# brendel-group/cl-ica

Hardware: AMD Instinct MI355X
Metric: training steps/sec (B=6144, n=10 MLP) (higher is better)
Workload: dtype f32 via f16x2 split (3 fp16 MFMA products of scaled two-piece operands, fp32 accumulate)

## Files before the change

cl_ica_amd/_lib.py:

```python
from __future__ import annotations

import ctypes as C
import os
import weakref
from typing import Dict, List, Optional, Tuple

import torch

_HERE = os.path.dirname(os.path.abspath(__file__))
LIB_PATH = os.environ.get("CLICA_LIB") or os.path.join(_HERE, "lib", "libclica_hip.so")

c_f32p = C.c_void_p
c_i64 = C.c_int64
c_i32 = C.c_int32
c_size = C.c_size_t


class LpLossDesc(C.Structure):
    _fields_ = [("B", c_i64), ("B3", c_i64), ("n", c_i32), ("p", C.c_float), ("tau", C.c_float),
                ("alpha", C.c_float), ("compat", c_i32), ("pow", c_i32), ("no_eps", c_i32)]


class AdamDesc(C.Structure):
    _fields_ = [("param", C.c_void_p), ("grad", C.c_void_p), ("exp_avg", C.c_void_p), ("exp_avg_sq", C.c_void_p), ("count", c_i64),
# ... 62 lines not shown
                                 c_f32p, c_i64, c_f32p, c_i64, C.c_void_p, c_size, C.c_void_p],
    "clica_dot_loss_bwd_sym_train": [C.POINTER(DotLossDesc), c_f32p, c_i64, c_f32p, c_i64, c_f32p, c_f32p, c_f32p, c_i64, c_f32p, C.c_void_p,
                                     C.c_void_p, c_size, C.c_void_p],
    "clica_linear_fwd": [c_f32p, c_i64, c_f32p, c_i64, c_f32p, c_f32p, c_i64, c_i64, c_i64, c_i64, c_i32, C.c_float, C.c_void_p],
    "clica_linear_dgrad": [c_f32p, c_i64, c_f32p, c_i64, c_f32p, c_i64, C.c_float, c_f32p, c_i64, c_i64, c_i64, c_i64, C.c_void_p],
    "clica_linear_wgrad_workspace_bytes": [c_i64, c_i64, c_i64, C.POINTER(c_size)],
    "clica_linear_plan": [c_i32, c_i64, c_i64, c_i64, C.POINTER(c_i32), C.POINTER(c_i32), C.POINTER(c_i32), C.POINTER(c_i32)],
    "clica_linear_wgrad": [c_f32p, c_i64, c_f32p, c_i64, c_f32p, c_i64, c_f32p, c_i64, c_i64, c_i64, c_i32, C.c_void_p, c_size, C.c_void_p],
    "clica_mlp_fwd": [c_f32p, c_i64, c_i64, c_i32, C.POINTER(C.c_void_p), C.POINTER(c_i64), C.POINTER(C.c_void_p),
                      C.POINTER(C.c_void_p), C.POINTER(c_i64), C.POINTER(c_i32), C.POINTER(c_i32), c_f32p, C.POINTER(C.c_void_p), C.c_float, C.c_void_p],
    "clica_mlp_fwd_mixed": [c_f32p, c_i64, c_i64, c_f32p, c_i32, C.c_float, c_f32p, c_i64, c_i32,
                            C.POINTER(C.c_void_p), C.POINTER(c_i64), C.POINTER(C.c_void_p),
                            C.POINTER(C.c_void_p), C.POINTER(c_i64), C.POINTER(c_i32), C.POINTER(c_i32), c_f32p, C.POINTER(C.c_void_p),
                            C.c_float, C.c_void_p],
    "clica_mlp_signmask_bytes": [c_i64, C.POINTER(c_size)],
    "clica_mlp_pack_split_bytes": [c_i32, C.POINTER(c_i32), C.POINTER(c_i32), c_i32, C.POINTER(c_size)],
    "clica_mlp_pack_split": [c_i32, C.POINTER(C.c_void_p), C.POINTER(c_i64), C.POINTER(c_i32), C.POINTER(c_i32), c_i32, C.c_void_p, C.c_void_p],
    "clica_mlp_pack_split_both": [c_i32, C.POINTER(C.c_void_p), C.POINTER(c_i64), C.POINTER(c_i32), C.POINTER(c_i32), C.c_void_p, C.c_void_p,
                                  C.c_void_p],
    "clica_mlp_planes_bytes": [c_i64, c_i32, c_i32, C.POINTER(c_size)],
    "clica_mlp_fwd_split": [c_f32p, c_i64, c_i64, c_f32p, c_i32, C.c_float, c_f32p, c_i64, c_i32, C.POINTER(C.c_void_p),
                            C.POINTER(C.c_void_p), C.POINTER(c_i64), C.POINTER(c_i32), C.POINTER(c_i32), C.c_void_p, C.POINTER(C.c_void_p),
                            C.POINTER(C.c_void_p), C.c_float, C.c_void_p],
    "clica_mlp_dgrad_split": [c_f32p, c_i64, c_i64, c_i32, C.POINTER(c_i32), C.POINTER(c_i32), C.c_void_p, C.POINTER(C.c_void_p),
                              C.POINTER(C.c_void_p), C.POINTER(c_i64), C.POINTER(C.c_void_p), C.c_float, C.c_void_p],
    "clica_mlp_wgrad_split_kind": [c_i32, c_i32, C.POINTER(c_i32)],
    "clica_mlp_planes_from_f32": [c_f32p, c_i64, c_i64, c_i32, c_i32, C.c_void_p, C.c_void_p],
    "clica_mlp_planes_from_f32_t": [c_f32p, c_i64, c_i64, c_i32, C.c_void_p, C.c_void_p],
    "clica_linear_split_fwd": [C.c_void_p, C.c_void_p, c_f32p, c_i64, c_i32, c_i32, c_i32, C.c_float, C.c_void_p, C.c_void_p, c_i32,
                               c_f32p, c_i64, C.c_void_p],
    "clica_linear_split_dgrad": [C.c_void_p, C.c_void_p, C.c_void_p, C.c_float, c_i64, c_i32, c_i32, C.c_void_p, C.c_void_p,
                                 c_f32p, c_i64, C.c_void_p],
    "clica_mlp_wgrad_split_workspace_bytes": [c_i64, c_i32, C.POINTER(c_i32), C.POINTER(c_i32), C.POINTER(c_size)],
    "clica_mlp_wgrad_split": [c_i64, c_i32, C.POINTER(C.c_void_p), C.POINTER(C.c_void_p), C.POINTER(C.c_void_p), C.POINTER(c_i64),
                              C.POINTER(C.c_void_p), C.POINTER(c_i64), C.POINTER(C.c_void_p), C.POINTER(c_i64), C.POINTER(C.c_void_p),
                              C.POINTER(c_i32), C.POINTER(c_i32), c_i32, C.c_void_p, c_size, C.c_void_p],
    "clica_split16_state_bytes": [C.POINTER(c_size)],
    "clica_split16_state_init": [C.c_void_p, C.c_void_p],
    "clica_split16_update": [C.c_void_p, c_i32, C.c_void_p],
    "clica_split16_read": [C.c_void_p, C.POINTER(c_i32), C.POINTER(c_i32), c_f32p, c_f32p, c_f32p, c_f32p, c_f32p, C.c_void_p],
    "clica_split16_clear_flags": [C.c_void_p, C.c_void_p],
    "clica_split16_guard": [C.c_void_p, C.POINTER(c_i32), C.POINTER(c_i32), C.POINTER(c_i32), C.POINTER(c_i32), C.c_void_p],
    "clica_split16_set_dp_poison": [C.c_void_p, C.c_void_p, C.c_void_p],
    "clica_split16_poison_export": [C.c_void_p, C.c_void_p, C.c_void_p],
    "clica_mlp_planes16_bytes": [c_i64, c_i32, c_i32, C.POINTER(c_size)],
    "clica_mlp_pack_split16_bytes": [c_i32, C.POINTER(c_i32), C.POINTER(c_i32), c_i32, C.POINTER(c_size)],
    "clica_mlp_pack_split16_both": [c_i32, C.POINTER(C.c_void_p), C.POINTER(c_i64), C.POINTER(c_i32), C.POINTER(c_i32), C.c_void_p, C.c_void_p,
                                    C.c_void_p, C.c_void_p],
    "clica_mlp_fwd_split16": [c_f32p, c_i64, c_i64, c_f32p, c_i32, C.c_float, c_f32p, c_i64, c_i32, C.POINTER(C.c_void_p),
                              C.POINTER(C.c_void_p), C.POINTER(c_i64), C.POINTER(c_i32), C.POINTER(c_i32), C.c_void_p, C.POINTER(C.c_void_p),
                              C.POINTER(C.c_void_p), C.c_float, C.c_void_p, C.c_void_p],
    "clica_mlp_dgrad_split16": [c_f32p, c_i64, c_i64, c_i32, C.POINTER(c_i32), C.POINTER(c_i32), C.c_void_p, C.POINTER(C.c_void_p),
                                C.POINTER(C.c_void_p), C.POINTER(c_i64), C.POINTER(C.c_void_p), C.c_float, C.c_void_p, C.c_void_p],
    "clica_mlp_wgrad_split16": [c_i64, c_i32, C.POINTER(C.c_void_p), C.POINTER(C.c_void_p), C.POINTER(C.c_void_p), C.POINTER(c_i64),
                                C.POINTER(C.c_void_p), C.POINTER(c_i64), C.POINTER(C.c_void_p), C.POINTER(c_i64), C.POINTER(C.c_void_p),
                                C.POINTER(c_i32), C.POINTER(c_i32), c_i32, C.c_void_p, C.POINTER(c_i32), C.POINTER(c_i32), C.c_void_p, c_size,
                                C.c_void_p],
    "clica_mlp_wgrad_split16_tail": [c_i64, c_i32, C.POINTER(C.c_void_p), C.POINTER(C.c_void_p), C.POINTER(C.c_void_p), C.POINTER(c_i64),
                                     C.POINTER(C.c_void_p), C.POINTER(c_i64), C.POINTER(C.c_void_p), C.POINTER(c_i64), C.POINTER(C.c_void_p),
                                     C.POINTER(c_i32), C.POINTER(c_i32), c_i32, C.c_void_p, C.POINTER(c_i32), C.POINTER(c_i32), c_i32, C.c_void_p, c_size,
                                     C.c_void_p],
    "clica_mlp_wgrad_split_adam": [c_i64, c_i32, C.POINTER(C.c_void_p), C.POINTER(C.c_void_p), C.POINTER(C.c_void_p), C.POINTER(c_i64),
                                   C.POINTER(C.c_void_p), C.POINTER(c_i64), C.POINTER(C.c_void_p), C.POINTER(c_i64), C.POINTER(C.c_void_p),
                                   C.POINTER(c_i32), C.POINTER(c_i32), C.c_void_p, C.POINTER(c_i32), C.POINTER(c_i32), C.POINTER(AdamDesc),
                                   c_i32, C.c_void_p, c_size, C.c_void_p],
    "clica_mlp_chain_tail_supported": [c_i32, C.POINTER(c_i32), C.POINTER(c_i32), C.POINTER(c_i32)],
# ... 180 lines not shown
```

cl_ica_amd/csrc/wgrad_split.hip:

```cpp
#include "common.h"
#include "planes.h"
#include "split16.h"
#include "wgrad_shared.h"
#include <algorithm>
#include <stdlib.h>

namespace clica {
namespace wsplit {

using gemm::MAXG;

typedef __bf16 bf16x8 __attribute__((ext_vector_type(8)));
typedef short s16x4 __attribute__((ext_vector_type(4)));
typedef float f32x16 __attribute__((ext_vector_type(16)));

#ifndef CLICA_WSPLIT_ABLATE
#define CLICA_WSPLIT_ABLATE 0
#endif
constexpr int STG = 4;
constexpr int UW = 8, UN = 4;
constexpr int THREADS = 512;
template <int AR> struct WArith;
template <> struct WArith<0> { static constexpr int NP = 3, NPROD = 6; static constexpr int PA[6] = {2, 0, 1, 1, 0, 0}, PB[6] = {0, 2, 1, 0, 1, 0}; };
template <> struct WArith<1> { static constexpr int NP = 2, NPROD = 3; static constexpr int PA[3] = {1, 0, 0}, PB[3] = {0, 1, 0}; };
template <int AR> constexpr int pieces_of() { return WArith<AR>::NP * (UW + UN); }
template <int AR> constexpr int stage_bytes_of() { return pieces_of<AR>() * 1024; }
constexpr size_t kLdsBytes = (size_t)STG * stage_bytes_of<0>();
template <int AR> constexpr size_t lds_bytes_of() { return (size_t)STG * stage_bytes_of<AR>(); }
typedef _Float16 f16x8 __attribute__((ext_vector_type(8)));

struct Prob {
  const char* A; const char* B;
  int fuA, fuB;
  float* C; int64_t ldc;
  float* dbslab;
  int M, N;
  int groups, gps;
  int gx, gy, a_wide;
  int n_big, rows_big;
  int epi;
  int leaky; float slope;
  const float* bias;
  const char* signT; int fuS;
  char* outT; int fuT;
  char* outN; int fuN;
  float* outF; int64_t ldf;
  const float* scaleA; const float* scaleB;
  s16::S16Tensor outS;
};
struct GroupArgs { int n, total; int first[MAXG + 1]; Prob p[MAXG]; };

__device__ __attribute__((aligned(16))) unsigned g_zero16[4] = {0u, 0u, 0u, 0u};

typedef __attribute__((address_space(3))) char* lds_ptr;
__device__ __forceinline__ void dma_1k(const char* lane_src, unsigned lds_off) {
#pragma clang diagnostic push
#pragma clang diagnostic ignored "-Winline-asm"
  asm volatile("s_mov_b32 m0, %1\n\ts_nop 0\n\tglobal_load_lds_dwordx4 %0, off" ::"v"(lane_src), "s"(lds_off) : "memory", "m0");
#pragma clang diagnostic pop
}
template <int N> __device__ __forceinline__ void wait_vm() {
  __builtin_amdgcn_s_waitcnt(0x0F70 | (N & 15) | ((N >> 4) << 14));
}
typedef unsigned u32x4 __attribute__((ext_vector_type(4)));
typedef unsigned u32x2 __attribute__((ext_vector_type(2)));
typedef u32x4 frag_t;
__device__ __forceinline__ frag_t read_frag(const char* p) {
  const u32x2 a = __builtin_bit_cast(u32x2, __builtin_amdgcn_ds_read_tr16_b64_v4i16((s16x4 __attribute__((address_space(3)))*)(lds_ptr)p));
  const u32x2 b = __builtin_bit_cast(u32x2, __builtin_amdgcn_ds_read_tr16_b64_v4i16((s16x4 __attribute__((address_space(3)))*)(lds_ptr)(p + 256)));
  return (frag_t){a.x, a.y, b.x, b.y};
}

template <int AR>
__device__ __forceinline__ f32x16 mfma32(const frag_t a, const frag_t b, const f32x16 c) {
  if constexpr (AR == 0) return __builtin_amdgcn_mfma_f32_32x32x16_bf16(__builtin_bit_cast(bf16x8, a), __builtin_bit_cast(bf16x8, b), c, 0, 0, 0);
  else return __builtin_amdgcn_mfma_f32_32x32x16_f16(__builtin_bit_cast(f16x8, a), __builtin_bit_cast(f16x8, b), c, 0, 0, 0);
}

#ifdef CLICA_WSPLIT_TRACE
__device__ unsigned long long* g_wstrace = nullptr;
#define WS_DECL unsigned long long ws_ts[16] = {0, 0, 0, 0, 0, 0, 0, 0, 0, 0, 0, 0, 0, 0, 0, 0}
#define WS_STAMP(ph) do { ws_ts[ph] = __builtin_readcyclecounter(); } while (0)
#define WS_STEP_STAMP(t, ph) do { if ((t) == 30) WS_STAMP(ph); } while (0)
// ... 424 lines not shown
    step(fa1, fb1, fa0, fb0, t + 1);
  }
  if (t < nt) step(fa0, fb0, fa1, fb1, t);
  WS_STAMP(2);

  const int m0 = by * BM, n0 = bx * BN;
  if constexpr (FUSED) {
    if constexpr (AR == 0) fused_epilogue<2>(g, acc, m0 + wm * 64, n0 + wn * 64, lane);
    else if constexpr (FUSED >= 16) fused_epilogue16_fast<2, FUSED>(g, acc, m0 + wm * 64, n0 + wn * 64, lane);
    else fused_epilogue16<2>(g, acc, m0 + wm * 64, n0 + wn * 64, lane);
    return;
  }
  float* Cbase = g.C + (int64_t)bz * g.M * g.ldc;
  float unscale = 1.f, unscale_db = 1.f;
  if constexpr (AR == 1) { unscale = 1.f / (*g.scaleA * *g.scaleB); unscale_db = 1.f / *g.scaleA; }
#pragma unroll
  for (int i = 0; i < 2; ++i) {
#pragma unroll
    for (int j = 0; j < 2; ++j) {
      const int col = n0 + wn * 64 + j * 32 + l31;
      const bool is_db = g.dbslab && col == g.N;
      if (col >= g.N && !is_db) continue;
      float* dst = is_db ? g.dbslab + (int64_t)bz * g.M : Cbase + col;
      const int64_t ld = is_db ? 1 : g.ldc;
#pragma unroll
      for (int r = 0; r < 16; ++r) {
        const int row = m0 + wm * 64 + i * 32 + (r & 3) + 8 * (r >> 2) + 4 * h;
        if (row >= g.M) continue;
        dst[row * ld] = AR == 1 ? acc[i][j][r] * (is_db ? unscale_db : unscale) : acc[i][j][r];
      }
    }
  }
  WS_STAMP(3);
  WS_FLUSH;
}

constexpr int STG2 = 3;
static_assert((size_t)STG2 * 3 * (UW + UW) * 1024 <= kLdsBytes && (size_t)STG2 * 2 * (UW + UW) * 1024 <= lds_bytes_of<1>(), "the big-tile stages must fit the launch's LDS");
template <int FUSED, int AR>
__device__ __forceinline__ void body_big(const Prob& g, const int bx, const int by, const int bz) {
  constexpr int NP = WArith<AR>::NP, NPROD = WArith<AR>::NPROD, PIECES2 = NP * (UW + UW), STAGE2_BYTES = PIECES2 * 1024;
  constexpr int NJ2 = PIECES2 / 8;
  constexpr int NMH = NPROD * 4;

  extern __shared__ __attribute__((aligned(16))) char smem[];
  const int lane = threadIdx.x & 63;
  const int wave = __builtin_amdgcn_readfirstlane(threadIdx.x >> 6);
  const int wm = wave >> 2, wn = wave & 3, h = lane >> 5, l31 = lane & 31;
  const int g0 = bz * g.gps;
  const int nt = min(g.groups, g0 + g.gps) - g0;
  WS_DECL;
  WS_STAMP(0);
  f32x16 acc[4][2];
#pragma unroll
  for (int i = 0; i < 4; ++i)
#pragma unroll
    for (int j = 0; j < 2; ++j)
#pragma unroll
      for (int r = 0; r < 16; ++r) acc[i][j][r] = 0.f;
  const unsigned lds0 = (unsigned)(size_t)(lds_ptr)smem;
  const char* src[NJ2]; int stride[NJ2];
#pragma unroll
  for (int j = 0; j < NJ2; ++j) {
    const int pi = wave + 8 * j;
    const bool is_a = pi < NP * UW;
    const int q = is_a ? pi : pi - NP * UW;
// ... 103 lines not shown
  }
  float* Cbase = g.C + (int64_t)bz * g.M * g.ldc;
  float unscale = 1.f, unscale_db = 1.f;
  if constexpr (AR == 1) { unscale = 1.f / (*g.scaleA * *g.scaleB); unscale_db = 1.f / *g.scaleA; }
#pragma unroll
  for (int i = 0; i < 4; ++i) {
#pragma unroll
    for (int j = 0; j < 2; ++j) {
      const int col = n0 + wn * 64 + j * 32 + l31;
      const bool is_db = g.dbslab && col == g.N;
      if (col >= g.N && !is_db) continue;
      float* dst = is_db ? g.dbslab + (int64_t)bz * g.M : Cbase + col;
      const int64_t ld = is_db ? 1 : g.ldc;
#pragma unroll
      for (int r = 0; r < 16; ++r) {
        const int row = m0 + wm * 128 + i * 32 + (r & 3) + 8 * (r >> 2) + 4 * h;
        if (row >= g.M) continue;
        dst[row * ld] = AR == 1 ? acc[i][j][r] * (is_db ? unscale_db : unscale) : acc[i][j][r];
      }
    }
  }
  WS_STAMP(3);
  WS_NOTE(11, 1000 + nt);
  WS_FLUSH;
}

__device__ __forceinline__ int xcd_contiguous(int b, int nwg) {
  const int xcd = b & 7, q = nwg >> 3, r = nwg & 7;
  return (xcd < r ? xcd * (q + 1) : r * (q + 1) + (xcd - r) * q) + (b >> 3);
}

template <int AR>
__global__ __launch_bounds__(THREADS) void wgrad_split_k(GroupArgs G) {
  const int id = xcd_contiguous(blockIdx.x, G.total);
  int q = 0;
#pragma unroll
  for (int i = 1; i < MAXG; ++i) q += (i < G.n && id >= G.first[i]) ? 1 : 0;
  const Prob& g = G.p[q];
  const int local = id - G.first[q];
  const int tiles = g.gx * g.gy;
  const int bz = local / tiles, t = local - bz * tiles;
  const int by = t / g.gx, bx = t - by * g.gx;
  if (g.a_wide == 2) body_big<false, AR>(g, bx, by, bz); else if (g.a_wide) body<true, false, AR>(g, bx, by, bz); else body<false, false, AR>(g, bx, by, bz);
}

template <int AR, int EPI = 1>
__global__ __launch_bounds__(THREADS) void gemm_split_k(GroupArgs G) {
  const Prob& g = G.p[0];
  if (g.a_wide == 3) {
    const int b = (int)blockIdx.x;
    if (b < g.n_big) {
      const int id = xcd_contiguous(b, g.n_big);
      const int by = id / g.gx, bx = id - by * g.gx;
      body_big<EPI, AR>(g, bx, by, 0);
    } else {
      const int id = xcd_contiguous(b - g.n_big, G.total - g.n_big);
      const int by = id / g.gx, bx = id - by * g.gx;
      body<false, EPI, AR>(g, bx, g.rows_big / 128 + by, 0);
    }
    return;
  }
  const int id = xcd_contiguous(blockIdx.x, G.total);
  const int by = id / g.gx, bx = id - by * g.gx;
  if (g.a_wide == 2) body_big<EPI, AR>(g, bx, by, 0); else if (g.a_wide) body<true, EPI, AR>(g, bx, by, 0); else body<false, EPI, AR>(g, bx, by, 0);
}

#ifdef CLICA_WSPLIT_TRACE
// ... 127 lines not shown
  float amax = 0.f;
  {
    const int phi = t >> 2, c = (t & 3) * 4;
    const int64_t row = (int64_t)u * 32 + phi; const int64_t f0 = g * 16 + c;
    float v[4] = {0.f, 0.f, 0.f, 0.f};
    if (live && row < M) {
      const float* src = X + row * ldx + f0;
      if (f0 + 3 < F && ((reinterpret_cast<uintptr_t>(src) & 15) == 0)) {
        const float4 x4 = *reinterpret_cast<const float4*>(src);
        v[0] = x4.x; v[1] = x4.y; v[2] = x4.z; v[3] = x4.w;
      } else {
#pragma unroll
        for (int e = 0; e < 4; ++e) if (f0 + e < F) v[e] = src[e];
      }
    }
    amax = fmaxf(fmaxf(fabsf(v[0]), fabsf(v[1])), fmaxf(fabsf(v[2]), fabsf(v[3])));
#pragma unroll
    for (int e = 0; e < 4; ++e) tile[half][c + e][phi] = v[e];
  }
  __syncthreads();
  if (live) {
    const int k = t >> 3, q = t & 7;
    unsigned hb[4], lb[4];
#pragma unroll
    for (int e = 0; e < 4; ++e) split16_hi_lo(tile[half][k][q * 4 + e] * sc, hb[e], lb[e]);
    const int sidx = q >> 2, c = (q & 3) * 4;
    char* dst = out + ((g * units + u) * 2) * 1024 + (k >> 2) * 256 + sidx * 128 + (k & 3) * 32 + c * 2;
    *reinterpret_cast<u32x2*>(dst) = (u32x2){hb[0] | (hb[1] << 16), hb[2] | (hb[3] << 16)};
    *reinterpret_cast<u32x2*>(dst + 1024) = (u32x2){lb[0] | (lb[1] << 16), lb[2] | (lb[3] << 16)};
  }
  s16::s16_commit_block_max(T, amax, red, blockIdx.x, gridDim.x);
}

struct Plan { int splits, gps, groups, tiles, n_tiny, tiny_splits; int64_t tiny_kps; int big_tiles; };
static void tile_shape(int32_t N, int32_t K, int* kind, int* gx, int* gy, bool with_db) {
  const int cols = K + (with_db ? 1 : 0);
  if (N > 128 && cols > 128) { *kind = 2; *gy = (int)ceil_div(N, 256); *gx = (int)ceil_div(cols, 256); return; }
  *kind = N >= K ? 1 : 0;
  const int bm = *kind ? 256 : 128, bn = *kind ? 128 : 256;
  *gy = (int)ceil_div(N, bm);
  *gx = (int)ceil_div(cols, bn);
}
static int problem_splits(const Plan& p, int kind) { return kind == 2 ? (int)ceil_div(p.groups, (int64_t)std::max(1, p.gps / 2)) : p.splits; }
static int problem_gps(const Plan& p, int kind) { return kind == 2 ? std::max(1, p.gps / 2) : p.gps; }
static Plan make_plan(int64_t Mrows, int n, const int32_t* N, const int32_t* K) {
  Plan p{};
  p.groups = (int)planes::groups_used(Mrows);
  for (int l = 0; l < n; ++l) {
    if (gemm::wgrad_tiny_shape(N[l], K[l])) { ++p.n_tiny; continue; }
    int kind, gx, gy; tile_shape(N[l], K[l], &kind, &gx, &gy, true);
    if (kind == 2) p.big_tiles += gx * gy; else p.tiles += gx * gy;
  }
  const int max_s = std::max(1, std::min(64, p.groups / (p.big_tiles ? 16 : 8)));
  double best = 1e300;
  p.splits = 1; p.gps = p.groups;
  for (int s = 1; s <= max_s && (p.tiles + p.big_tiles) > 0; ++s) {
    int gps = (int)ceil_div(p.groups, s);
    if (p.big_tiles) gps = (gps + 1) & ~1;
    const int sp = (int)ceil_div(p.groups, gps);
    const int sp_big = p.big_tiles ? (int)ceil_div(p.groups, gps / 2) : 0;
    const int64_t items = (int64_t)p.tiles * sp + (int64_t)p.big_tiles * sp_big;
    const int64_t rounds = ceil_div(items, kNumCU);
    const double cost = (double)rounds * (16.0 * gps + 48.0) + 8.0 * sp + (p.big_tiles ? 4.0 * sp_big : 0.0);
    if (cost < best) { best = cost; p.splits = sp; p.gps = gps; }
  }
  if (p.n_tiny > 0) gemm::wgrad_tiny_plan(Mrows, p.n_tiny, &p.tiny_splits, &p.tiny_kps);
  return p;
}
static int layer_splits(const Plan& p, int32_t N, int32_t K) {
  if (gemm::wgrad_tiny_shape(N, K)) return p.tiny_splits;
  int kind, gx, gy; tile_shape(N, K, &kind, &gx, &gy, true);
  return problem_splits(p, kind);
}
bool chain_tail_supported(int n_layers, const int32_t* N, const int32_t* K) {
  if (n_layers < 2) return false;
  const int l = n_layers - 1;
  return gemm::wgrad_tiny_shape(N[0], K[0]) && gemm::wgrad_tiny_shape(N[l], K[l]) && K[0] <= 15 && N[0] <= 128 && N[l] <= 16 && K[l] <= 127;
}
static int tail_splits(int64_t Mrows) { return (int)ceil_div(Mrows, (int64_t)kChainRows); }
static size_t slabs_alloc(const Plan& p, int64_t Mrows, int n, const int32_t* N, const int32_t* K, int l) {
  size_t sp = (size_t)layer_splits(p, N[l], K[l]);
  if ((l == 0 || l == n - 1) && chain_tail_supported(n, N, K)) sp = std::max(sp, (size_t)tail_splits(Mrows));
  return sp;
}
static size_t ws_layout(const Plan& p, int64_t Mrows, int n, const int32_t* N, const int32_t* K, size_t* slab_off, size_t* db_off) {
  size_t off = 0;
  for (int l = 0; l < n; ++l) {
    const size_t sp = slabs_alloc(p, Mrows, n, N, K, l);
    if (slab_off) slab_off[l] = off;
    off += align_up(sp * N[l] * K[l] * sizeof(float), 256);
    if (db_off) db_off[l] = off;
    off += align_up(sp * N[l] * sizeof(float), 256);
  }
  return off;
}
int chain_tail_slabs(int64_t M, int n_layers, const int32_t* N, const int32_t* K, void* workspace, size_t workspace_bytes,
                     float** slab_first, float** db_first, float** slab_last, float** db_last) {
  if (!chain_tail_supported(n_layers, N, K) || n_layers > MAXG) { set_error("chain tail: these layer shapes are not supported"); return CLICA_E_INVALID; }
  size_t slab_off[MAXG], db_off[MAXG];
  const size_t need = ws_layout(make_plan(M, n_layers, N, K), M, n_layers, N, K, slab_off, db_off);
  if (!workspace || need > workspace_bytes) { set_error("chain tail: weight-gradient workspace %zu < %zu", workspace_bytes, need); return CLICA_E_WORKSPACE; }
  char* w = reinterpret_cast<char*>(workspace);
  *slab_first = reinterpret_cast<float*>(w + slab_off[0]); *db_first = reinterpret_cast<float*>(w + db_off[0]);
  *slab_last = reinterpret_cast<float*>(w + slab_off[n_layers - 1]); *db_last = reinterpret_cast<float*>(w + db_off[n_layers - 1]);
  return CLICA_OK;
}

}
}

using namespace clica;
using namespace clica::wsplit;

extern "C" int clica_mlp_planes_from_f32(const float* X, int64_t ldx, int64_t M, int32_t width, int32_t ones_column, void* planes_out,
                                         clica_stream_t stream) {
  CLICA_CHECK_ARG(X && planes_out && M > 0 && width >= 1 && ldx >= width, "clica_mlp_planes_from_f32: bad argument");
  CLICA_CHECK_ARG((reinterpret_cast<uintptr_t>(planes_out) & 15) == 0, "clica_mlp_planes_from_f32: plane buffer must be 16-byte aligned");
  const int units = planes::units(width, ones_column);
  const int64_t groups = planes::groups_alloc(M);
  hipLaunchKernelGGL(planes_from_f32_k, dim3((unsigned)ceil_div(groups * units, 2)), dim3(256), 0, as_stream(stream),
                     X, ldx, M, (int)width, ones_column ? 1 : 0, units, reinterpret_cast<char*>(planes_out), groups);
  return launch_status("clica_mlp_planes_from_f32");
}

extern "C" int clica_mlp_wgrad_split_kind(int32_t N, int32_t K, int32_t* kind) {
  CLICA_CHECK_ARG(kind && N >= 1 && K >= 1, "clica_mlp_wgrad_split_kind: bad argument");
  *kind = gemm::wgrad_tiny_shape(N, K) ? 1 : 0;
  return CLICA_OK;
}

extern "C" int clica_mlp_wgrad_split_workspace_bytes(int64_t M, int32_t n_layers, const int32_t* N, const int32_t* K, size_t* bytes) {
  CLICA_CHECK_ARG(bytes && N && K && M > 0 && n_layers >= 1 && n_layers <= MAXG, "clica_mlp_wgrad_split_workspace_bytes: bad argument");
  for (int l = 0; l < n_layers; ++l) CLICA_CHECK_ARG(N[l] >= 1 && K[l] >= 1, "clica_mlp_wgrad_split_workspace_bytes: layer %d: bad size", l);
  *bytes = ws_layout(make_plan(M, n_layers, N, K), M, n_layers, N, K, nullptr, nullptr);
  return CLICA_OK;
}

typedef s16::Split16State Split16Scales;

static int mlp_wgrad_split_impl(int64_t M, int32_t n_layers, const void* const* dZ_planes, const void* const* X_planes,
                                const float* const* dZ, const int64_t* lddz, const float* const* X, const int64_t* ldx,
                                float* const* dW, const int64_t* lddw, float* const* db, const int32_t* N, const int32_t* K,
                                int32_t accumulate, const void* state16, const int32_t* a_index, const int32_t* d_index,
                                void* workspace, size_t workspace_bytes, clica_stream_t stream, const clica_adam_desc* adam = nullptr,
                                int tail_slabs = 0) {
  CLICA_CHECK_ARG(dZ_planes && X_planes && dZ && lddz && X && ldx && dW && lddw && db && N && K && workspace && M > 0,
                  "clica_mlp_wgrad_split: NULL pointer / empty batch");
  CLICA_CHECK_ARG(n_layers >= 1 && n_layers <= MAXG, "clica_mlp_wgrad_split: %d layers (1..%d supported)", n_layers, MAXG);
  CLICA_CHECK_ARG(!tail_slabs || chain_tail_supported(n_layers, N, K), "clica_mlp_wgrad_split_adam: tail_slabs set for shapes the chain's tail does not cover");
  const Plan p = make_plan(M, n_layers, N, K);
  size_t slab_off[MAXG], db_off[MAXG];
  const size_t need = ws_layout(p, M, n_layers, N, K, slab_off, db_off);
  if (need > workspace_bytes) { set_error("clica_mlp_wgrad_split: workspace %zu < %zu", workspace_bytes, need); return CLICA_E_WORKSPACE; }
  hipStream_t st = as_stream(stream);
  GroupArgs G{};
  gemm::ReduceGroupArgs R{};
  gemm::TinyArgs T{};
  R.n = n_layers; R.accumulate = accumulate ? 1 : 0;
  if (adam) {
    CLICA_CHECK_ARG(adam->param && adam->grad && adam->exp_avg && adam->exp_avg_sq && adam->step_dev && adam->count > 0 && !accumulate,
                    "clica_mlp_wgrad_split_adam: NULL arena / accumulate set");
    CLICA_CHECK_ARG((((uintptr_t)adam->param | (uintptr_t)adam->grad | (uintptr_t)adam->exp_avg | (uintptr_t)adam->exp_avg_sq) & 15) == 0,
                    "clica_mlp_wgrad_split_adam: arenas must be 16-byte aligned");
    CLICA_CHECK_ARG(adam->t_offset == 0 || adam->t_offset == 1, "clica_mlp_wgrad_split_adam: t_offset must be 0 or 1");
    CLICA_CHECK_ARG(!adam->split16_state || (adam->n_layers >= 1 && adam->n_layers <= 8), "clica_mlp_wgrad_split_adam: bad layer count");
    int64_t covered = 0;
    for (int l = 0; l < n_layers; ++l) {
      CLICA_CHECK_ARG(dW[l] && db[l] && lddw[l] == K[l], "clica_mlp_wgrad_split_adam: layer %d: dW must be contiguous, db present", l);
      CLICA_CHECK_ARG(dW[l] >= adam->grad && dW[l] + (int64_t)N[l] * K[l] <= adam->grad + adam->count && db[l] >= adam->grad &&
                      db[l] + N[l] <= adam->grad + adam->count, "clica_mlp_wgrad_split_adam: layer %d: dW / db outside the gradient arena", l);
      covered += (int64_t)N[l] * K[l] + N[l];
    }
    CLICA_CHECK_ARG(adam->count - covered >= 0 && adam->count - covered <= 8 * (int64_t)n_layers,
                    "clica_mlp_wgrad_split_adam: the arena holds %lld elements, the layers cover %lld", (long long)adam->count, (long long)covered);
    R.adam.p = adam->param; R.adam.m = adam->exp_avg; R.adam.v = adam->exp_avg_sq; R.adam.gbase = adam->grad;
    R.adam.lr = adam->lr; R.adam.b1 = adam->beta1; R.adam.b2 = adam->beta2; R.adam.eps = adam->eps; R.adam.gscale = adam->grad_scale;
    R.adam.step_dev = adam->step_dev; R.adam.t_offset = adam->t_offset;
    R.adam.s16_state = adam->split16_state; R.adam.s16_layers = adam->n_layers;
  }
  int item = 0, rblock = 0, ng = 0;
  for (int l = 0; l < n_layers; ++l) {
    CLICA_CHECK_ARG(dW[l] && N[l] >= 1 && K[l] >= 1 && lddw[l] >= K[l], "clica_mlp_wgrad_split: layer %d: bad argument", l);
    const bool tiny = gemm::wgrad_tiny_shape(N[l], K[l]);
    const bool from_chain = tail_slabs && (l == 0 || l == n_layers - 1);
    const int sp = from_chain ? tail_splits(M) : layer_splits(p, N[l], K[l]);
    float* slab = (float*)((char*)workspace + slab_off[l]);
    float* dbslab = (float*)((char*)workspace + db_off[l]);
    if (from_chain) {
      CLICA_CHECK_ARG(db[l], "clica_mlp_wgrad_split_adam: layer %d: tail slabs need a bias gradient", l);
    } else if (tiny) {
      CLICA_CHECK_ARG(dZ[l] && X[l] && lddz[l] >= N[l] && ldx[l] >= K[l],
                      "clica_mlp_wgrad_split: layer %d (%d x %d) takes the fp32 tiny-dimension kernel: fp32 operands required", l, N[l], K[l]);
      gemm::Args g{};
      g.A = dZ[l]; g.lda = lddz[l]; g.B = X[l]; g.ldb = ldx[l]; g.C = slab; g.ldc = K[l]; g.M = N[l]; g.N = K[l]; g.Kc = M;
      g.k_per_split = p.tiny_kps; g.dbias_slab = db[l] ? dbslab : nullptr;
      T.p[T.n++] = g;
    } else {
      CLICA_CHECK_ARG(dZ_planes[l] && X_planes[l], "clica_mlp_wgrad_split: layer %d (%d x %d) needs the bf16 plane copies of both "
                      "operands (clica_mlp_fwd_split / clica_mlp_dgrad_split with a plane buffer)", l, N[l], K[l]);
      CLICA_CHECK_ARG(((reinterpret_cast<uintptr_t>(dZ_planes[l]) | reinterpret_cast<uintptr_t>(X_planes[l])) & 15) == 0,
                      "clica_mlp_wgrad_split: layer %d: plane buffers must be 16-byte aligned", l);
      Prob& g = G.p[ng];
      g.A = reinterpret_cast<const char*>(dZ_planes[l]); g.fuA = planes::units(N[l], 0);
      g.B = reinterpret_cast<const char*>(X_planes[l]); g.fuB = planes::units(K[l], 1);
      g.C = slab; g.ldc = K[l]; g.dbslab = db[l] ? dbslab : nullptr; g.M = N[l]; g.N = K[l];
      tile_shape(N[l], K[l], &g.a_wide, &g.gx, &g.gy, true);
      g.groups = p.groups; g.gps = problem_gps(p, g.a_wide);
      if (state16) {
        const Split16Scales* st16 = reinterpret_cast<const Split16Scales*>(state16);
        CLICA_CHECK_ARG(a_index && d_index && a_index[l] >= 0 && a_index[l] < 9 && d_index[l] >= 0 && d_index[l] < 9,
                        "clica_mlp_wgrad_split16: layer %d: scale index out of range", l);
        g.scaleA = &st16->sD[d_index[l]]; g.scaleB = &st16->sA[a_index[l]];
      }
      G.first[ng] = item; item += g.gx * g.gy * sp;
      ++ng;
    }
    rblock += gemm::slab_reduce_entry(R, l, rblock, sp, slab, dbslab, dW[l], lddw[l], db[l], N[l], K[l]);
  }
  G.n = ng; G.first[ng] = G.total = item; R.first[n_layers] = rblock;
  if (T.n > 0) {
    int rct = gemm::launch_wgrad_tiny(T, p.tiny_splits, st);
    if (rct) return rct;
  }
  if (ng > 0) {
    if (state16) {
      static bool once = ((void)hipFuncSetAttribute(reinterpret_cast<const void*>(wgrad_split_k<1>), hipFuncAttributeMaxDynamicSharedMemorySize, (int)lds_bytes_of<1>()), true);
      (void)once;
      hipLaunchKernelGGL(wgrad_split_k<1>, dim3((unsigned)item), dim3(THREADS), lds_bytes_of<1>(), st, G);
    } else {
      static bool once = ((void)hipFuncSetAttribute(reinterpret_cast<const void*>(wgrad_split_k<0>), hipFuncAttributeMaxDynamicSharedMemorySize, (int)kLdsBytes), true);
      (void)once;
      hipLaunchKernelGGL(wgrad_split_k<0>, dim3((unsigned)item), dim3(THREADS), kLdsBytes, st, G);
    }
    int rc = launch_status("clica_mlp_wgrad_split");
    if (rc) return rc;
  }
  return gemm::launch_slab_reduce_group(R, rblock, st);
}

extern "C" int clica_mlp_wgrad_split(int64_t M, int32_t n_layers, const void* const* dZ_planes, const void* const* X_planes,
                                     const float* const* dZ, const int64_t* lddz, const float* const* X, const int64_t* ldx,
                                     float* const* dW, const int64_t* lddw, float* const* db, const int32_t* N, const int32_t* K,
                                     int32_t accumulate, void* workspace, size_t workspace_bytes, clica_stream_t stream) {
  return mlp_wgrad_split_impl(M, n_layers, dZ_planes, X_planes, dZ, lddz, X, ldx, dW, lddw, db, N, K, accumulate, nullptr, nullptr, nullptr,
                              workspace, workspace_bytes, stream);
}
extern "C" int clica_mlp_wgrad_split16(int64_t M, int32_t n_layers, const void* const* dZ_planes, const void* const* X_planes,
                                       const float* const* dZ, const int64_t* lddz, const float* const* X, const int64_t* ldx,
                                       float* const* dW, const int64_t* lddw, float* const* db, const int32_t* N, const int32_t* K,
                                       int32_t accumulate, const void* state, const int32_t* a_index, const int32_t* d_index,
                                       void* workspace, size_t workspace_bytes, clica_stream_t stream) {
  CLICA_CHECK_ARG(state && a_index && d_index, "clica_mlp_wgrad_split16: NULL state / index arrays");
// ... 220 lines not shown
```

include/clica.h:

```cpp
#ifndef CLICA_H
#define CLICA_H

#include <stddef.h>
#include <stdint.h>

#ifdef __cplusplus
extern "C" {
#endif

#define CLICA_OK 0
#define CLICA_E_INVALID (-1)
#define CLICA_E_WORKSPACE (-2)
#define CLICA_E_HIP (-3)

typedef void* clica_stream_t;

const char* clica_last_error(void);
int clica_set_tuning(const char* key, int32_t value);
int clica_abort_capture(clica_stream_t stream);
int clica_version(void);

typedef struct clica_lp_loss_desc {
  int64_t B;
  int64_t B3;
// ... 126 lines not shown
int clica_mlp_pack(int32_t n_layers, const float* const* W, const int64_t* ldw, const int32_t* N, const int32_t* K,
                   int32_t transpose, float* packed, clica_stream_t stream);
int clica_mlp_pack_both(int32_t n_layers, const float* const* W, const int64_t* ldw, const int32_t* N, const int32_t* K,
                        float* packed_fwd, float* packed_bwd, clica_stream_t stream);
int clica_mlp_dgrad(const float* dY, int64_t lddy, int64_t M, int32_t n_links,
                    const int32_t* N, const int32_t* K, const float* packed,
                    const float* const* act, const int64_t* ldact, const uint64_t* const* signmask,
                    float* const* out, const int64_t* ldo, float slope, clica_stream_t stream);
int clica_mlp_planes_bytes(int64_t M, int32_t width, int32_t ones_column, size_t* bytes);
int clica_mlp_pack_split_bytes(int32_t n_layers, const int32_t* N, const int32_t* K, int32_t transpose, size_t* bytes);
int clica_mlp_pack_split(int32_t n_layers, const float* const* W, const int64_t* ldw, const int32_t* N, const int32_t* K,
                         int32_t transpose, void* packed, clica_stream_t stream);
int clica_mlp_pack_split_both(int32_t n_layers, const float* const* W, const int64_t* ldw, const int32_t* N, const int32_t* K,
                              void* packed_fwd, void* packed_bwd, clica_stream_t stream);
int clica_mlp_fwd_split(const float* X, int64_t ldx, int64_t M, const float* mix_W, int32_t mix_layers, float mix_slope,
                        float* x_out, int64_t ldxo, int32_t n_layers, const float* const* bias,
                        float* const* out, const int64_t* ldo, const int32_t* N, const int32_t* K,
                        const void* packed_split, uint64_t* const* signmask, void* const* planes, float slope,
                        clica_stream_t stream);
int clica_mlp_dgrad_split(const float* dY, int64_t lddy, int64_t M, int32_t n_links, const int32_t* N, const int32_t* K,
                          const void* packed_split, const uint64_t* const* signmask,
                          float* const* out, const int64_t* ldo, void* const* planes, float slope, clica_stream_t stream);
int clica_mlp_wgrad_split_kind(int32_t N, int32_t K, int32_t* kind);
int clica_mlp_planes_from_f32(const float* X, int64_t ldx, int64_t M, int32_t width, int32_t ones_column, void* planes_out,
                              clica_stream_t stream);
int clica_mlp_planes_from_f32_t(const float* X, int64_t ldx, int64_t M, int32_t width, void* planes_out, clica_stream_t stream);
int clica_linear_split_fwd(const void* xT_planes, const void* wT_planes, const float* bias, int64_t M, int32_t N, int32_t K,
                           int32_t leaky, float slope, void* yT_planes, void* yN_planes, int32_t yN_ones,
                           float* Y, int64_t ldy, clica_stream_t stream);
int clica_linear_split_dgrad(const void* dzT_planes, const void* wN_planes, const void* actT_planes, float slope,
                             int64_t M, int32_t N, int32_t K, void* dxT_planes, void* dxN_planes,
                             float* dX, int64_t lddx, clica_stream_t stream);
int clica_mlp_wgrad_split_workspace_bytes(int64_t M, int32_t n_layers, const int32_t* N, const int32_t* K, size_t* bytes);
int clica_mlp_wgrad_split(int64_t M, int32_t n_layers, const void* const* dZ_planes, const void* const* X_planes,
                          const float* const* dZ, const int64_t* lddz, const float* const* X, const int64_t* ldx,
                          float* const* dW, const int64_t* lddw, float* const* db, const int32_t* N, const int32_t* K,
                          int32_t accumulate, void* workspace, size_t workspace_bytes, clica_stream_t stream);

int clica_split16_state_bytes(size_t* bytes);
int clica_split16_state_init(void* state, clica_stream_t stream);
int clica_split16_update(void* state, int32_t n_layers, clica_stream_t stream);
int clica_split16_read(const void* state, int32_t* flags, int32_t* updates, float* scales_a, float* scales_d, float* scales_w,
                       float* last_scales_a, float* last_scales_d, clica_stream_t stream);
int clica_split16_clear_flags(void* state, clica_stream_t stream);
int clica_split16_guard(const void* state, int32_t* flags, int32_t* skipped, int32_t* updates, int32_t* poisoned, clica_stream_t stream);
int clica_split16_set_dp_poison(void* state, const float* slot, clica_stream_t stream);
int clica_split16_poison_export(const void* state, float* slot, clica_stream_t stream);
int clica_mlp_planes16_bytes(int64_t M, int32_t width, int32_t ones_column, size_t* bytes);
int clica_mlp_pack_split16_bytes(int32_t n_layers, const int32_t* N, const int32_t* K, int32_t transpose, size_t* bytes);
int clica_mlp_pack_split16_both(int32_t n_layers, const float* const* W, const int64_t* ldw, const int32_t* N, const int32_t* K,
                                void* packed_fwd, void* packed_bwd, void* state, clica_stream_t stream);
int clica_mlp_fwd_split16(const float* X, int64_t ldx, int64_t M, const float* mix_W, int32_t mix_layers, float mix_slope,
                          float* x_out, int64_t ldxo, int32_t n_layers, const float* const* bias,
                          float* const* out, const int64_t* ldo, const int32_t* N, const int32_t* K,
                          const void* packed_split16, uint64_t* const* signmask, void* const* planes, float slope,
                          void* state, clica_stream_t stream);
int clica_mlp_dgrad_split16(const float* dY, int64_t lddy, int64_t M, int32_t n_links, const int32_t* N, const int32_t* K,
                            const void* packed_split16, const uint64_t* const* signmask,
                            float* const* out, const int64_t* ldo, void* const* planes, float slope, void* state, clica_stream_t stream);
int clica_mlp_wgrad_split16(int64_t M, int32_t n_layers, const void* const* dZ_planes, const void* const* X_planes,
                            const float* const* dZ, const int64_t* lddz, const float* const* X, const int64_t* ldx,
                            float* const* dW, const int64_t* lddw, float* const* db, const int32_t* N, const int32_t* K,
                            int32_t accumulate, const void* state, const int32_t* a_index, const int32_t* d_index,
                            void* workspace, size_t workspace_bytes, clica_stream_t stream);

int clica_mse_loss_workspace_bytes(int64_t M, int32_t n, size_t* bytes);
// ... 201 lines not shown
```

Baseline: 2805.

## Plan wgrad split-K per tile kind with a cost model and a lead-first dispatch

Replaces the coupled split-K planner with one that picks the number of K-splits separately for small and large tile kinds. In the split16 arithmetic path it scores each choice with per-item cycle costs taken from traces, and the kernel then dispatches the slower kind first (lead) with its own XCD-contiguous block mapping. Plans are cached per shape in a thread-local, and a query API exposes the chosen plan. The aim is better load balance across CUs and less padding in the last round, at the price of hard-coded cost constants and a larger workspace, since slabs are sized as the maximum over both plans.

```diff
diff --git a/cl_ica_amd/_lib.py b/cl_ica_amd/_lib.py
--- a/cl_ica_amd/_lib.py
+++ b/cl_ica_amd/_lib.py
@@ -118,6 +118,8 @@
     "clica_linear_split_dgrad": [C.c_void_p, C.c_void_p, C.c_void_p, C.c_float, c_i64, c_i32, c_i32, C.c_void_p, C.c_void_p,
                                  c_f32p, c_i64, C.c_void_p],
     "clica_mlp_wgrad_split_workspace_bytes": [c_i64, c_i32, C.POINTER(c_i32), C.POINTER(c_i32), C.POINTER(c_size)],
+    "clica_mlp_wgrad_split_plan": [c_i64, c_i32, C.POINTER(c_i32), C.POINTER(c_i32), c_i32, C.POINTER(c_i32), C.POINTER(c_i32),
+                                   C.POINTER(c_i32), C.POINTER(c_i32), C.POINTER(c_i64), C.POINTER(c_i64), C.POINTER(c_i64), C.POINTER(c_i64)],
     "clica_mlp_wgrad_split": [c_i64, c_i32, C.POINTER(C.c_void_p), C.POINTER(C.c_void_p), C.POINTER(C.c_void_p), C.POINTER(c_i64),
                               C.POINTER(C.c_void_p), C.POINTER(c_i64), C.POINTER(C.c_void_p), C.POINTER(c_i64), C.POINTER(C.c_void_p),
                               C.POINTER(c_i32), C.POINTER(c_i32), c_i32, C.c_void_p, c_size, C.c_void_p],
diff --git a/cl_ica_amd/csrc/wgrad_split.hip b/cl_ica_amd/csrc/wgrad_split.hip
--- a/cl_ica_amd/csrc/wgrad_split.hip
+++ b/cl_ica_amd/csrc/wgrad_split.hip
@@ -48,7 +48,7 @@
   const float* scaleA; const float* scaleB;
   s16::S16Tensor outS;
 };
-struct GroupArgs { int n, total; int first[MAXG + 1]; Prob p[MAXG]; };
+struct GroupArgs { int n, total; int first[MAXG + 1]; Prob p[MAXG]; int lead; };
 
 __device__ __attribute__((aligned(16))) unsigned g_zero16[4] = {0u, 0u, 0u, 0u};
 
@@ -539,6 +539,7 @@
     }
   }
   WS_STAMP(3);
+  WS_NOTE(11, nt);
   WS_FLUSH;
 }
 
@@ -708,7 +709,8 @@
 
 template <int AR>
 __global__ __launch_bounds__(THREADS) void wgrad_split_k(GroupArgs G) {
-  const int id = xcd_contiguous(blockIdx.x, G.total);
+  const int b = (int)blockIdx.x;
+  const int id = b < G.lead ? xcd_contiguous(b, G.lead) : G.lead + xcd_contiguous(b - G.lead, G.total - G.lead);
   int q = 0;
 #pragma unroll
   for (int i = 1; i < MAXG; ++i) q += (i < G.n && id >= G.first[i]) ? 1 : 0;
@@ -902,7 +904,14 @@
   s16::s16_commit_block_max(T, amax, red, blockIdx.x, gridDim.x);
 }
 
-struct Plan { int splits, gps, groups, tiles, n_tiny, tiny_splits; int64_t tiny_kps; int big_tiles; };
+struct Plan {
+  int groups;
+  int tiles[2];
+  int sp[2], gps[2];
+  int lead;
+  double item_cycles[2];
+  int n_tiny, tiny_splits; int64_t tiny_kps;
+};
 static void tile_shape(int32_t N, int32_t K, int* kind, int* gx, int* gy, bool with_db) {
   const int cols = K + (with_db ? 1 : 0);
   if (N > 128 && cols > 128) { *kind = 2; *gy = (int)ceil_div(N, 256); *gx = (int)ceil_div(cols, 256); return; }
@@ -911,28 +920,64 @@
   *gy = (int)ceil_div(N, bm);
   *gx = (int)ceil_div(cols, bn);
 }
-static int problem_splits(const Plan& p, int kind) { return kind == 2 ? (int)ceil_div(p.groups, (int64_t)std::max(1, p.gps / 2)) : p.splits; }
-static int problem_gps(const Plan& p, int kind) { return kind == 2 ? std::max(1, p.gps / 2) : p.gps; }
-static Plan make_plan(int64_t Mrows, int n, const int32_t* N, const int32_t* K) {
+static int plan_kind(int tile_kind) { return tile_kind == 2 ? 1 : 0; }
+struct ItemCost { bool traced; double fixed[2], step[2]; };
+constexpr ItemCost kItemCost[2] = {
+   {false, {0.0, 0.0}, {0.0, 0.0}},
+   {true, {4494.0 + 6792.0, 7594.0 + 15954.0}, {122796.0 / 86.0, 96060.0 / 43.0}},
+};
+constexpr double kSlabSplitCycles[2] = {8.0 * 1428.0 / 16.0, 4.0 * 1428.0 / 16.0};
+static double item_cycles(int arith, int kind, int steps) { return kItemCost[arith].fixed[kind] + steps * kItemCost[arith].step[kind]; }
+
+static Plan coupled_plan(Plan p, int64_t Mrows, int max_s) {
+  double best = 1e300;
+  p.lead = -1;
+  for (int k = 0; k < 2; ++k) { p.sp[k] = 1; p.gps[k] = p.groups; }
+  for (int s = 1; s <= max_s && (p.tiles[0] + p.tiles[1]) > 0; ++s) {
+    int gps = (int)ceil_div(p.groups, s);
+    if (p.tiles[1]) gps = (gps + 1) & ~1;
+    const int sp = (int)ceil_div(p.groups, gps);
+    const int gps_big = std::max(1, gps / 2);
+    const int sp_big = p.tiles[1] ? (int)ceil_div(p.groups, gps_big) : 0;
+    const int64_t rounds = ceil_div((int64_t)p.tiles[0] * sp + (int64_t)p.tiles[1] * sp_big, kNumCU);
+    const double cost = (double)rounds * (16.0 * gps + 48.0) + 8.0 * sp + (p.tiles[1] ? 4.0 * sp_big : 0.0);
+    if (cost < best) { best = cost; p.sp[0] = sp; p.gps[0] = gps; p.sp[1] = std::max(1, sp_big); p.gps[1] = gps_big; }
+  }
+  if (p.n_tiny > 0) gemm::wgrad_tiny_plan(Mrows, p.n_tiny, &p.tiny_splits, &p.tiny_kps);
+  return p;
+}
+static Plan make_plan(int64_t Mrows, int n, const int32_t* N, const int32_t* K, int arith) {
   Plan p{};
   p.groups = (int)planes::groups_used(Mrows);
   for (int l = 0; l < n; ++l) {
     if (gemm::wgrad_tiny_shape(N[l], K[l])) { ++p.n_tiny; continue; }
     int kind, gx, gy; tile_shape(N[l], K[l], &kind, &gx, &gy, true);
-    if (kind == 2) p.big_tiles += gx * gy; else p.tiles += gx * gy;
-  }
-  const int max_s = std::max(1, std::min(64, p.groups / (p.big_tiles ? 16 : 8)));
-  double best = 1e300;
-  p.splits = 1; p.gps = p.groups;
-  for (int s = 1; s <= max_s && (p.tiles + p.big_tiles) > 0; ++s) {
-    int gps = (int)ceil_div(p.groups, s);
-    if (p.big_tiles) gps = (gps + 1) & ~1;
-    const int sp = (int)ceil_div(p.groups, gps);
-    const int sp_big = p.big_tiles ? (int)ceil_div(p.groups, gps / 2) : 0;
-    const int64_t items = (int64_t)p.tiles * sp + (int64_t)p.big_tiles * sp_big;
-    const int64_t rounds = ceil_div(items, kNumCU);
-    const double cost = (double)rounds * (16.0 * gps + 48.0) + 8.0 * sp + (p.big_tiles ? 4.0 * sp_big : 0.0);
-    if (cost < best) { best = cost; p.splits = sp; p.gps = gps; }
+    p.tiles[plan_kind(kind)] += gx * gy;
+  }
+  const int max_s = std::max(1, std::min(64, p.groups / (p.tiles[1] ? 16 : 8)));
+  if (!kItemCost[arith].traced) return coupled_plan(p, Mrows, max_s);
+  const int max_of[2] = {p.tiles[0] ? max_s : 1, p.tiles[1] ? 2 * max_s : 1};
+  double best = 1e300; int best_slabs = 0;
+  for (int k = 0; k < 2; ++k) { p.sp[k] = 1; p.gps[k] = p.groups; }
+  for (int s0 = 1; s0 <= max_of[0] && (p.tiles[0] + p.tiles[1]) > 0; ++s0) {
+    const int gps0 = (int)ceil_div(p.groups, s0);
+    if ((int)ceil_div(p.groups, gps0) != s0) continue;
+    for (int s1 = 1; s1 <= max_of[1]; ++s1) {
+      const int gps1 = (int)ceil_div(p.groups, s1);
+      if ((int)ceil_div(p.groups, gps1) != s1) continue;
+      const double t[2] = {p.tiles[0] ? item_cycles(arith, 0, gps0) : 0.0, p.tiles[1] ? item_cycles(arith, 1, gps1) : 0.0};
+      const int64_t items[2] = {(int64_t)p.tiles[0] * s0, (int64_t)p.tiles[1] * s1};
+      const int lead = t[1] >= t[0] ? 1 : 0;
+      const int64_t rounds = ceil_div(items[0] + items[1], (int64_t)kNumCU);
+      const int64_t lead_rounds = std::min(rounds, ceil_div(items[lead], (int64_t)kNumCU));
+      const double cost = (double)lead_rounds * t[lead] + (double)(rounds - lead_rounds) * t[1 - lead] +
+                          (p.tiles[0] ? kSlabSplitCycles[0] * s0 : 0.0) + (p.tiles[1] ? kSlabSplitCycles[1] * s1 : 0.0);
+      const int slabs = (p.tiles[0] ? s0 : 0) + (p.tiles[1] ? s1 : 0);
+      if (cost < best || (cost == best && slabs < best_slabs)) {
+        best = cost; best_slabs = slabs; p.lead = lead;
+        p.sp[0] = s0; p.gps[0] = gps0; p.sp[1] = s1; p.gps[1] = gps1; p.item_cycles[0] = t[0]; p.item_cycles[1] = t[1];
+      }
+    }
   }
   if (p.n_tiny > 0) gemm::wgrad_tiny_plan(Mrows, p.n_tiny, &p.tiny_splits, &p.tiny_kps);
   return p;
@@ -940,7 +985,22 @@
 static int layer_splits(const Plan& p, int32_t N, int32_t K) {
   if (gemm::wgrad_tiny_shape(N, K)) return p.tiny_splits;
   int kind, gx, gy; tile_shape(N, K, &kind, &gx, &gy, true);
-  return problem_splits(p, kind);
+  return p.sp[plan_kind(kind)];
+}
+struct Dispatch { int n, n_lead; int layer[MAXG]; int first[MAXG + 1]; };
+static Dispatch dispatch_order(const Plan& p, int n, const int32_t* N, const int32_t* K) {
+  Dispatch d{};
+  for (int pass = 0; pass < 2; ++pass) {
+    for (int l = 0; l < n; ++l) {
+      if (gemm::wgrad_tiny_shape(N[l], K[l])) continue;
+      int kind, gx, gy; tile_shape(N[l], K[l], &kind, &gx, &gy, true);
+      if (p.lead >= 0 ? (plan_kind(kind) == p.lead) != (pass == 0) : pass != 0) continue;
+      d.layer[d.n] = l; d.first[d.n + 1] = d.first[d.n] + gx * gy * p.sp[plan_kind(kind)];
+      ++d.n;
+    }
+    if (pass == 0) d.n_lead = d.first[d.n];
+  }
+  return d;
 }
 bool chain_tail_supported(int n_layers, const int32_t* N, const int32_t* K) {
   if (n_layers < 2) return false;
@@ -948,15 +1008,30 @@
   return gemm::wgrad_tiny_shape(N[0], K[0]) && gemm::wgrad_tiny_shape(N[l], K[l]) && K[0] <= 15 && N[0] <= 128 && N[l] <= 16 && K[l] <= 127;
 }
 static int tail_splits(int64_t Mrows) { return (int)ceil_div(Mrows, (int64_t)kChainRows); }
-static size_t slabs_alloc(const Plan& p, int64_t Mrows, int n, const int32_t* N, const int32_t* K, int l) {
-  size_t sp = (size_t)layer_splits(p, N[l], K[l]);
+struct Plans { Plan of[2]; };
+static Plans make_plans(int64_t Mrows, int n, const int32_t* N, const int32_t* K) {
+  struct Key { int64_t M; int n; int32_t N[MAXG], K[MAXG]; };
+  thread_local Key last{};
+  thread_local Plans kept{};
+  Key k{};
+  k.M = Mrows; k.n = n;
+  for (int l = 0; l < n && l < MAXG; ++l) { k.N[l] = N[l]; k.K[l] = K[l]; }
+  bool same = last.M == k.M && last.n == k.n;
+  for (int l = 0; same && l < MAXG; ++l) same = last.N[l] == k.N[l] && last.K[l] == k.K[l];
+  if (same) return kept;
+  kept = Plans{{make_plan(Mrows, n, N, K, 0), make_plan(Mrows, n, N, K, 1)}};
+  last = k;
+  return kept;
+}
+static size_t slabs_alloc(const Plans& ps, int64_t Mrows, int n, const int32_t* N, const int32_t* K, int l) {
+  size_t sp = (size_t)std::max(layer_splits(ps.of[0], N[l], K[l]), layer_splits(ps.of[1], N[l], K[l]));
   if ((l == 0 || l == n - 1) && chain_tail_supported(n, N, K)) sp = std::max(sp, (size_t)tail_splits(Mrows));
   return sp;
 }
-static size_t ws_layout(const Plan& p, int64_t Mrows, int n, const int32_t* N, const int32_t* K, size_t* slab_off, size_t* db_off) {
+static size_t ws_layout(const Plans& ps, int64_t Mrows, int n, const int32_t* N, const int32_t* K, size_t* slab_off, size_t* db_off) {
   size_t off = 0;
   for (int l = 0; l < n; ++l) {
-    const size_t sp = slabs_alloc(p, Mrows, n, N, K, l);
+    const size_t sp = slabs_alloc(ps, Mrows, n, N, K, l);
     if (slab_off) slab_off[l] = off;
     off += align_up(sp * N[l] * K[l] * sizeof(float), 256);
     if (db_off) db_off[l] = off;
@@ -968,7 +1043,7 @@
                      float** slab_first, float** db_first, float** slab_last, float** db_last) {
   if (!chain_tail_supported(n_layers, N, K) || n_layers > MAXG) { set_error("chain tail: these layer shapes are not supported"); return CLICA_E_INVALID; }
   size_t slab_off[MAXG], db_off[MAXG];
-  const size_t need = ws_layout(make_plan(M, n_layers, N, K), M, n_layers, N, K, slab_off, db_off);
+  const size_t need = ws_layout(make_plans(M, n_layers, N, K), M, n_layers, N, K, slab_off, db_off);
   if (!workspace || need > workspace_bytes) { set_error("chain tail: weight-gradient workspace %zu < %zu", workspace_bytes, need); return CLICA_E_WORKSPACE; }
   char* w = reinterpret_cast<char*>(workspace);
   *slab_first = reinterpret_cast<float*>(w + slab_off[0]); *db_first = reinterpret_cast<float*>(w + db_off[0]);
@@ -1002,7 +1077,33 @@
 extern "C" int clica_mlp_wgrad_split_workspace_bytes(int64_t M, int32_t n_layers, const int32_t* N, const int32_t* K, size_t* bytes) {
   CLICA_CHECK_ARG(bytes && N && K && M > 0 && n_layers >= 1 && n_layers <= MAXG, "clica_mlp_wgrad_split_workspace_bytes: bad argument");
   for (int l = 0; l < n_layers; ++l) CLICA_CHECK_ARG(N[l] >= 1 && K[l] >= 1, "clica_mlp_wgrad_split_workspace_bytes: layer %d: bad size", l);
-  *bytes = ws_layout(make_plan(M, n_layers, N, K), M, n_layers, N, K, nullptr, nullptr);
+  *bytes = ws_layout(make_plans(M, n_layers, N, K), M, n_layers, N, K, nullptr, nullptr);
+  return CLICA_OK;
+}
+
+extern "C" int clica_mlp_wgrad_split_plan(int64_t M, int32_t n_layers, const int32_t* N, const int32_t* K, int32_t arith,
+                                          int32_t* splits, int32_t* steps, int32_t* first_item, int32_t* items,
+                                          int64_t* slab_offset, int64_t* db_offset, int64_t* slab_count, int64_t* summary) {
+  CLICA_CHECK_ARG(N && K && splits && steps && first_item && items && slab_offset && db_offset && slab_count && summary && M > 0 &&
+                  n_layers >= 1 && n_layers <= MAXG && (arith == 0 || arith == 1), "clica_mlp_wgrad_split_plan: bad argument");
+  for (int l = 0; l < n_layers; ++l) CLICA_CHECK_ARG(N[l] >= 1 && K[l] >= 1, "clica_mlp_wgrad_split_plan: layer %d: bad size", l);
+  const Plans plans = make_plans(M, n_layers, N, K);
+  const Plan& p = plans.of[arith];
+  size_t so[MAXG], dbo[MAXG];
+  const size_t bytes = ws_layout(plans, M, n_layers, N, K, so, dbo);
+  for (int l = 0; l < n_layers; ++l) {
+    splits[l] = layer_splits(p, N[l], K[l]); steps[l] = 0; first_item[l] = -1; items[l] = 0;
+    slab_offset[l] = (int64_t)so[l]; db_offset[l] = (int64_t)dbo[l]; slab_count[l] = (int64_t)slabs_alloc(plans, M, n_layers, N, K, l);
+  }
+  const Dispatch d = dispatch_order(p, n_layers, N, K);
+  for (int q = 0; q < d.n; ++q) {
+    const int l = d.layer[q];
+    int kind, gx, gy; tile_shape(N[l], K[l], &kind, &gx, &gy, true);
+    steps[l] = p.gps[plan_kind(kind)]; first_item[l] = d.first[q]; items[l] = d.first[q + 1] - d.first[q];
+  }
+  summary[0] = d.first[d.n]; summary[1] = d.n_lead; summary[2] = p.lead;
+  summary[3] = (int64_t)p.item_cycles[0]; summary[4] = (int64_t)p.item_cycles[1];
+  summary[5] = (int64_t)bytes; summary[6] = p.groups; summary[7] = kNumCU;
   return CLICA_OK;
 }
 
@@ -1018,9 +1119,10 @@
                   "clica_mlp_wgrad_split: NULL pointer / empty batch");
   CLICA_CHECK_ARG(n_layers >= 1 && n_layers <= MAXG, "clica_mlp_wgrad_split: %d layers (1..%d supported)", n_layers, MAXG);
   CLICA_CHECK_ARG(!tail_slabs || chain_tail_supported(n_layers, N, K), "clica_mlp_wgrad_split_adam: tail_slabs set for shapes the chain's tail does not cover");
-  const Plan p = make_plan(M, n_layers, N, K);
+  const Plans plans = make_plans(M, n_layers, N, K);
+  const Plan& p = plans.of[state16 ? 1 : 0];
   size_t slab_off[MAXG], db_off[MAXG];
-  const size_t need = ws_layout(p, M, n_layers, N, K, slab_off, db_off);
+  const size_t need = ws_layout(plans, M, n_layers, N, K, slab_off, db_off);
   if (need > workspace_bytes) { set_error("clica_mlp_wgrad_split: workspace %zu < %zu", workspace_bytes, need); return CLICA_E_WORKSPACE; }
   hipStream_t st = as_stream(stream);
   GroupArgs G{};
@@ -1048,7 +1150,8 @@
     R.adam.step_dev = adam->step_dev; R.adam.t_offset = adam->t_offset;
     R.adam.s16_state = adam->split16_state; R.adam.s16_layers = adam->n_layers;
   }
-  int item = 0, rblock = 0, ng = 0;
+  Prob of_layer[MAXG];
+  int rblock = 0;
   for (int l = 0; l < n_layers; ++l) {
     CLICA_CHECK_ARG(dW[l] && N[l] >= 1 && K[l] >= 1 && lddw[l] >= K[l], "clica_mlp_wgrad_split: layer %d: bad argument", l);
     const bool tiny = gemm::wgrad_tiny_shape(N[l], K[l]);
@@ -1070,24 +1173,25 @@
                       "operands (clica_mlp_fwd_split / clica_mlp_dgrad_split with a plane buffer)", l, N[l], K[l]);
       CLICA_CHECK_ARG(((reinterpret_cast<uintptr_t>(dZ_planes[l]) | reinterpret_cast<uintptr_t>(X_planes[l])) & 15) == 0,
                       "clica_mlp_wgrad_split: layer %d: plane buffers must be 16-byte aligned", l);
-      Prob& g = G.p[ng];
+      Prob& g = of_layer[l] = Prob{};
       g.A = reinterpret_cast<const char*>(dZ_planes[l]); g.fuA = planes::units(N[l], 0);
       g.B = reinterpret_cast<const char*>(X_planes[l]); g.fuB = planes::units(K[l], 1);
       g.C = slab; g.ldc = K[l]; g.dbslab = db[l] ? dbslab : nullptr; g.M = N[l]; g.N = K[l];
       tile_shape(N[l], K[l], &g.a_wide, &g.gx, &g.gy, true);
-      g.groups = p.groups; g.gps = problem_gps(p, g.a_wide);
+      g.groups = p.groups; g.gps = p.gps[plan_kind(g.a_wide)];
       if (state16) {
         const Split16Scales* st16 = reinterpret_cast<const Split16Scales*>(state16);
         CLICA_CHECK_ARG(a_index && d_index && a_index[l] >= 0 && a_index[l] < 9 && d_index[l] >= 0 && d_index[l] < 9,
                         "clica_mlp_wgrad_split16: layer %d: scale index out of range", l);
         g.scaleA = &st16->sD[d_index[l]]; g.scaleB = &st16->sA[a_index[l]];
       }
-      G.first[ng] = item; item += g.gx * g.gy * sp;
-      ++ng;
     }
     rblock += gemm::slab_reduce_entry(R, l, rblock, sp, slab, dbslab, dW[l], lddw[l], db[l], N[l], K[l]);
   }
-  G.n = ng; G.first[ng] = G.total = item; R.first[n_layers] = rblock;
+  const Dispatch d = dispatch_order(p, n_layers, N, K);
+  for (int q = 0; q < d.n; ++q) { G.p[q] = of_layer[d.layer[q]]; G.first[q] = d.first[q]; }
+  const int ng = d.n, item = d.first[d.n];
+  G.n = ng; G.first[ng] = G.total = item; G.lead = d.n_lead; R.first[n_layers] = rblock;
   if (T.n > 0) {
     int rct = gemm::launch_wgrad_tiny(T, p.tiny_splits, st);
     if (rct) return rct;
diff --git a/include/clica.h b/include/clica.h
--- a/include/clica.h
+++ b/include/clica.h
@@ -182,6 +182,9 @@
                              int64_t M, int32_t N, int32_t K, void* dxT_planes, void* dxN_planes,
                              float* dX, int64_t lddx, clica_stream_t stream);
 int clica_mlp_wgrad_split_workspace_bytes(int64_t M, int32_t n_layers, const int32_t* N, const int32_t* K, size_t* bytes);
+int clica_mlp_wgrad_split_plan(int64_t M, int32_t n_layers, const int32_t* N, const int32_t* K, int32_t arith,
+                               int32_t* splits, int32_t* steps, int32_t* first_item, int32_t* items,
+                               int64_t* slab_offset, int64_t* db_offset, int64_t* slab_count, int64_t* summary);
 int clica_mlp_wgrad_split(int64_t M, int32_t n_layers, const void* const* dZ_planes, const void* const* X_planes,
                           const float* const* dZ, const int64_t* lddz, const float* const* X, const int64_t* ldx,
                           float* const* dW, const int64_t* lddw, float* const* db, const int32_t* N, const int32_t* K,
```

Result: no change. 2823, median of 6 (+0.6%).
